# XuyangBai/D3Feat

Measured on NVIDIA H100. Metric: points/sec through KPFCNN encoder, higher is better.
Workload: dtype f32

## Files before the change

d3feat_b200/csrc/kpconv.cu:

```cuda
#include <stdlib.h>

#include "ops.cuh"

namespace d3f {


constexpr int kS1Warps = 4;
constexpr int kWStride = 20;
constexpr int kKMax = 16;

struct Stage1Params {
  const float* q;
  const float4* s4;
  const int* idx;
  const float* feat;
  int count_nn;
  const float* Kp;
  const float* offsets;
  const float* modulations;
  int Nq, Ns, H, Cin;
  int n0, n1;
  const int* order;
  float extent;
  float inv_scale;
// ... 200 lines not shown
__device__ __forceinline__ float sqrt_approx(float x) {
  float r;
  asm("sqrt.approx.ftz.f32 %0, %1;" : "=f"(r) : "f"(x));
  return r;
}

template <int CPL, int QPW, bool DEFORM>
__global__ void __launch_bounds__(kS1Warps * 32, CPL == 4 ? 4 : 6) kpconv_stage1_v2_kernel(Stage1Params p) {
  const int Ns_ = dyn_rows(p.Ns, p.ns_dev), n1_ = min(p.n1, dyn_rows(p.Nq, p.nq_dev));
  constexpr int K = 15, KP = 16;
  constexpr int LPQ = 32 / QPW;
  static_assert(CPL == 2 || CPL == 4, "channels per lane");
  __shared__ __align__(16) float wts[kS1Warps][32 * kWStride];
  __shared__ float kp_s[kS1Warps][QPW][KP * 3];
  const int lane = threadIdx.x & 31, warp = threadIdx.x >> 5;
  const int sub = lane / LPQ, sl = lane % LPQ;
  const int nfirst = p.n0 + (blockIdx.x * kS1Warps + warp) * QPW;
  if (nfirst >= n1_) return;
  const int n = nfirst + sub;
  const bool qvalid = n < n1_;
  const int nslot = qvalid ? n : nfirst;
  const int nq = p.order ? p.order[nslot] : nslot;

  for (int t = sl; t < KP * 3; t += LPQ) {
    float v = t < K * 3 ? p.Kp[t] : 0.f;
    if (DEFORM && t < K * 3) v += p.offsets[(size_t)nq * K * 3 + t];
    kp_s[warp][sub][t] = v;
  }
  const float qx = p.q[3 * (size_t)nq], qy = p.q[3 * (size_t)nq + 1], qz = p.q[3 * (size_t)nq + 2];
  const int* row = p.idx + (size_t)nq * p.H;
  const float ext2 = p.extent * p.extent;
  const unsigned gshift = (unsigned)(sub * LPQ);
  const unsigned gmask = LPQ == 32 ? 0xffffffffu : ((1u << LPQ) - 1u);
  float* wq = &wts[warp][sub * LPQ * kWStride];
  __syncwarp();

  int nn_count = 0;
  constexpr int c_step = LPQ * CPL;
  for (int c0 = 0; c0 < p.Cin; c0 += c_step) {
    float2 acc[KP / 2][CPL];
#pragma unroll
    for (int j = 0; j < KP / 2; ++j)
#pragma unroll
      for (int v = 0; v < CPL; ++v) acc[j][v] = make_float2(0.f, 0.f);
    const int c = c0 + sl * CPL;

    for (int h0 = 0; h0 < p.H; h0 += LPQ) {
      const int h = h0 + sl;
      int id = (h < p.H) ? row[h] : Ns_;
      if (id < 0 || id > Ns_) id = Ns_;
      const bool real = id < Ns_;
      const float4 sp = __ldg(&p.s4[id]);
      const float rx = sp.x - qx, ry = sp.y - qy, rz = sp.z - qz;
      float w[KP];
      float dmin = 3.0e38f;
      int kmin = 0;
      bool in_range = false;
#pragma unroll
      for (int k = 0; k < K; ++k) {
        float dx = rx - kp_s[warp][sub][3 * k], dy = ry - kp_s[warp][sub][3 * k + 1], dz = rz - kp_s[warp][sub][3 * k + 2];
        float d2 = dx * dx + dy * dy + dz * dz;
        if (d2 < dmin) { dmin = d2; kmin = k; }
        in_range = in_range || (d2 < ext2);
        float wk;
        if (p.influence == D3F_INFLUENCE_LINEAR) wk = fmaxf(1.f - sqrt_approx(d2 + 1e-10f) * p.inv_scale, 0.f);
        else if (p.influence == D3F_INFLUENCE_GAUSSIAN) wk = __expf(-d2 * p.gauss_inv);
        else wk = DEFORM ? (d2 < ext2 ? 1.f : 0.f) : 1.f;
        w[k] = wk;
      }
      w[K] = 0.f;
      if (p.closest) {
#pragma unroll
        for (int k = 0; k < K; ++k) w[k] = (k == kmin) ? w[k] : 0.f;
      }
      const bool keep = real && qvalid && (!DEFORM || in_range);
#pragma unroll
      for (int kq = 0; kq < KP / 4; ++kq)
        *reinterpret_cast<float4*>(&wq[sl * kWStride + 4 * kq]) =
            keep ? make_float4(w[4 * kq], w[4 * kq + 1], w[4 * kq + 2], w[4 * kq + 3]) : make_float4(0.f, 0.f, 0.f, 0.f);
      if (c0 == 0 && p.count_nn) nn_count += __popc((__ballot_sync(0xffffffffu, sp.w > 0.f) >> gshift) & gmask);
      unsigned m = (__ballot_sync(0xffffffffu, keep) >> gshift) & gmask;
      int cnt = __popc(m);
      if (QPW >= 2) cnt = max(cnt, __shfl_xor_sync(0xffffffffu, cnt, 16));
      if (QPW >= 4) cnt = max(cnt, __shfl_xor_sync(0xffffffffu, cnt, 8));
      __syncwarp();

      constexpr int kUnroll = CPL == 4 ? 2 : 4;
      for (int it = 0; it < cnt; it += kUnroll) {
        int hh[kUnroll];
        float f[kUnroll][CPL];
#pragma unroll
        for (int u = 0; u < kUnroll; ++u) {
          const bool act = m != 0;
          hh[u] = act ? __ffs(m) - 1 : 0;
          m &= m - 1;
          const int idh = __shfl_sync(0xffffffffu, id, (int)gshift + hh[u]);
          const float* fp = p.feat + (size_t)idh * p.Cin + c;
          if (CPL == 4) {
            float4 t = act ? __ldg(reinterpret_cast<const float4*>(fp)) : make_float4(0.f, 0.f, 0.f, 0.f);
            f[u][0] = t.x; f[u][1] = t.y; f[u][2 % CPL] = t.z; f[u][3 % CPL] = t.w;
          } else {
            float2 t = act ? __ldg(reinterpret_cast<const float2*>(fp)) : make_float2(0.f, 0.f);
            f[u][0] = t.x; f[u][1] = t.y;
          }
        }
#pragma unroll
        for (int u = 0; u < kUnroll; ++u) {
          const float4* wp = reinterpret_cast<const float4*>(&wq[hh[u] * kWStride]);
          float2 wpair[KP / 2];
#pragma unroll
          for (int kq = 0; kq < KP / 4; ++kq) {
            float4 t = wp[kq];
            wpair[2 * kq] = make_float2(t.x, t.y);
            wpair[2 * kq + 1] = make_float2(t.z, t.w);
          }
#pragma unroll
          for (int v = 0; v < CPL; ++v) {
            const float2 fd = make_float2(f[u][v], f[u][v]);
#pragma unroll
            for (int j = 0; j < KP / 2; ++j) acc[j][v] = ffma2(wpair[j], fd, acc[j][v]);
          }
        }
      }
      __syncwarp();
    }

    if (qvalid) {
      float* dst = p.wf + (size_t)(n - p.n0) * K * p.Cin + c;
#pragma unroll
      for (int k = 0; k < K; ++k) {
        const float mod = (DEFORM && p.modulations) ? p.modulations[(size_t)nq * K + k] : 1.f;
        float o[CPL];
#pragma unroll
        for (int v = 0; v < CPL; ++v) o[v] = ((k & 1) ? acc[k / 2][v].y : acc[k / 2][v].x) * mod;
        if (CPL == 4) *reinterpret_cast<float4*>(dst + (size_t)k * p.Cin) = make_float4(o[0], o[1], o[2 % CPL], o[3 % CPL]);
        else *reinterpret_cast<float2*>(dst + (size_t)k * p.Cin) = make_float2(o[0], o[1]);
      }
    }
  }
  if (p.inv_nn != nullptr && qvalid && sl == 0) p.inv_nn[n - p.n0] = 1.f / (float)max(nn_count, 1);
}

__device__ __forceinline__ void mma_tf32(float (&c)[4], const unsigned (&a)[4], unsigned b0, unsigned b1) {
  asm volatile("mma.sync.aligned.m16n8k8.row.col.f32.tf32.tf32.f32 {%0,%1,%2,%3}, {%4,%5,%6,%7}, {%8,%9}, {%0,%1,%2,%3};"
               : "+f"(c[0]), "+f"(c[1]), "+f"(c[2]), "+f"(c[3])
               : "r"(a[0]), "r"(a[1]), "r"(a[2]), "r"(a[3]), "r"(b0), "r"(b1));
}
__device__ __forceinline__ void split3(float x, unsigned& hi, unsigned& lo) {
  hi = (__float_as_uint(x) + 0x1000u) & 0xFFFFE000u;
  lo = __float_as_uint(x - __uint_as_float(hi));
}


template <int NT>
__global__ void __launch_bounds__(kS1Warps * 32, NT == 4 ? 8 : (NT == 8 ? 5 : 3))
kpconv_stage1_fast_kernel(Stage1Params p) {
  const int Ns_ = dyn_rows(p.Ns, p.ns_dev), n1_ = min(p.n1, dyn_rows(p.Nq, p.nq_dev));
  constexpr int K = 15;
  static_assert(NT % 4 == 0, "one float4 per four n-tiles");
  const int lane = threadIdx.x & 31, warp = threadIdx.x >> 5;
  const int g = lane >> 2, t = lane & 3;
  const int n = p.n0 + blockIdx.x * kS1Warps + warp;
  if (n >= n1_) return;
  const int kA = g, kB = g + 8;
  const bool validB = kB < K;
  const float kax = p.Kp[3 * kA], kay = p.Kp[3 * kA + 1], kaz = p.Kp[3 * kA + 2];
  const float kbx = validB ? p.Kp[3 * kB] : 1e6f, kby = validB ? p.Kp[3 * kB + 1] : 1e6f,
              kbz = validB ? p.Kp[3 * kB + 2] : 1e6f;
  const int qid = p.order ? p.order[n] : n;
  const float qx = p.q[3 * (size_t)qid], qy = p.q[3 * (size_t)qid + 1], qz = p.q[3 * (size_t)qid + 2];
  const int* row = p.idx + (size_t)qid * p.H + t;
  const float inv_scale = p.inv_scale;
  const unsigned Ns = (unsigned)Ns_;
  const unsigned Cin = (unsigned)p.Cin;
  int cnt = 0;

  constexpr int CCH = NT * 8;
  for (int c0 = blockIdx.y * CCH; c0 < p.Cin; c0 += gridDim.y * CCH) {
    float acc[NT][4];
#pragma unroll
    for (int i = 0; i < NT; ++i) acc[i][0] = acc[i][1] = acc[i][2] = acc[i][3] = 0.f;
    const float* fcol = p.feat + c0 + NT * g;
    asm volatile("" : "+l"(fcol));

    unsigned ida_n = Ns, idb_n = Ns;
    if (t < p.H) ida_n = (unsigned)__ldg(row);
    if (t + 4 < p.H) idb_n = (unsigned)__ldg(row + 4);
    for (int h0 = 0; h0 < p.H; h0 += 8) {
      const unsigned ida = min(ida_n, Ns);
      const unsigned idb = min(idb_n, Ns);
      ida_n = Ns;
      idb_n = Ns;
      if (h0 + 8 + t < p.H) ida_n = (unsigned)__ldg(row + h0 + 8);
      if (h0 + 12 + t < p.H) idb_n = (unsigned)__ldg(row + h0 + 12);
      const float4 spa = __ldg(&p.s4[ida]), spb = __ldg(&p.s4[idb]);
      float fa[NT], fb[NT];
#pragma unroll
      for (int v = 0; v < NT; v += 4) {
        float4 x = make_float4(0.f, 0.f, 0.f, 0.f), y = make_float4(0.f, 0.f, 0.f, 0.f);
        if (ida < Ns) x = __ldg(reinterpret_cast<const float4*>(fcol + (size_t)(ida * Cin) + v));
        if (idb < Ns) y = __ldg(reinterpret_cast<const float4*>(fcol + (size_t)(idb * Cin) + v));
        fa[v] = x.x; fa[v + 1] = x.y; fa[v + 2] = x.z; fa[v + 3] = x.w;
        fb[v] = y.x; fb[v + 1] = y.y; fb[v + 2] = y.z; fb[v + 3] = y.w;
      }
      if (c0 == 0) cnt += (spa.w > 0.f ? 1 : 0) + (spb.w > 0.f ? 1 : 0);
      const float rax = spa.x - qx, ray = spa.y - qy, raz = spa.z - qz;
      const float rbx = spb.x - qx, rby = spb.y - qy, rbz = spb.z - qz;
      auto weight = [&](float rx, float ry, float rz, float kx, float ky, float kz) {
        const float dx = rx - kx, dy = ry - ky, dz = rz - kz;
        const float d2 = fmaf(dz, dz, fmaf(dy, dy, fmaf(dx, dx, 1e-10f)));
        return fmaxf(fmaf(-sqrt_approx(d2), inv_scale, 1.f), 0.f);
      };
      unsigned ah[4], al[4];
      split3(weight(rax, ray, raz, kax, kay, kaz), ah[0], al[0]);
      split3(weight(rax, ray, raz, kbx, kby, kbz), ah[1], al[1]);
      split3(weight(rbx, rby, rbz, kax, kay, kaz), ah[2], al[2]);
      split3(weight(rbx, rby, rbz, kbx, kby, kbz), ah[3], al[3]);
#pragma unroll
      for (int i = 0; i < NT; ++i) {
        unsigned bh0, bl0, bh1, bl1;
        split3(fa[i], bh0, bl0);
        split3(fb[i], bh1, bl1);
        mma_tf32(acc[i], ah, bh0, bh1);
        mma_tf32(acc[i], al, bh0, bh1);
        mma_tf32(acc[i], ah, bl0, bl1);
      }
    }

    float* dst = p.wf + (size_t)(n - p.n0) * K * p.Cin + c0 + 2 * NT * t;
#pragma unroll
    for (int v = 0; v < NT; v += 4) {
      *reinterpret_cast<float4*>(dst + (size_t)kA * p.Cin + v) = make_float4(acc[v][0], acc[v + 1][0], acc[v + 2][0], acc[v + 3][0]);
      *reinterpret_cast<float4*>(dst + (size_t)kA * p.Cin + NT + v) = make_float4(acc[v][1], acc[v + 1][1], acc[v + 2][1], acc[v + 3][1]);
      if (validB) {
        *reinterpret_cast<float4*>(dst + (size_t)kB * p.Cin + v) = make_float4(acc[v][2], acc[v + 1][2], acc[v + 2][2], acc[v + 3][2]);
        *reinterpret_cast<float4*>(dst + (size_t)kB * p.Cin + NT + v) = make_float4(acc[v][3], acc[v + 1][3], acc[v + 2][3], acc[v + 3][3]);
      }
    }
  }
  if (p.inv_nn != nullptr && blockIdx.y == 0) {
    cnt += __shfl_xor_sync(0xffffffffu, cnt, 1);
    cnt += __shfl_xor_sync(0xffffffffu, cnt, 2);
    if (lane == 0) p.inv_nn[n - p.n0] = 1.f / (float)max(cnt, 1);
  }
}

__device__ __forceinline__ uint32_t s1_smem_u32(const void* p) { return (uint32_t)__cvta_generic_to_shared(p); }
__device__ __forceinline__ void s1_cp_async16(uint32_t dst, const void* src, bool valid) {
  const int sz = valid ? 16 : 0;
  asm volatile("cp.async.cg.shared.global [%0], [%1], 16, %2;" ::"r"(dst), "l"(src), "r"(sz) : "memory");
}
__device__ __forceinline__ float4 s1_lds128(uint32_t addr) {
  float4 v;
  asm volatile("ld.shared.v4.f32 {%0, %1, %2, %3}, [%4];" : "=f"(v.x), "=f"(v.y), "=f"(v.z), "=f"(v.w) : "r"(addr));
  return v;
}
template <int NT>
__device__ __forceinline__ int s1_swz(int r3) {
  return NT == 4 ? 2 * r3 : (NT == 8 ? ((r3 & 1) | ((r3 & 2) << 1)) : r3);
}

template <int NT>
__global__ void __launch_bounds__(kS1Warps * 32, NT == 4 ? 8 : (NT == 8 ? 5 : 3))
kpconv_stage1_staged_kernel(Stage1Params p) {
  constexpr int K = 15;
  constexpr int ROWB = NT * 32;
  constexpr int BUFB = 8 * ROWB + 128;
  __shared__ __align__(128) unsigned char stage_sm[kS1Warps][2][BUFB];
  const int Ns_ = dyn_rows(p.Ns, p.ns_dev), n1_ = min(p.n1, dyn_rows(p.Nq, p.nq_dev));
  const int lane = threadIdx.x & 31, warp = threadIdx.x >> 5;
  const int g = lane >> 2, t = lane & 3;
  const int n = p.n0 + blockIdx.x * kS1Warps + warp;
  if (n >= n1_) return;
  const int kA = g, kB = g + 8;
  const bool validB = kB < K;
  const float kax = p.Kp[3 * kA], kay = p.Kp[3 * kA + 1], kaz = p.Kp[3 * kA + 2];
  const float kbx = validB ? p.Kp[3 * kB] : 1e6f, kby = validB ? p.Kp[3 * kB + 1] : 1e6f,
              kbz = validB ? p.Kp[3 * kB + 2] : 1e6f;
  const int qid = p.order ? p.order[n] : n;
  const float qx = p.q[3 * (size_t)qid], qy = p.q[3 * (size_t)qid + 1], qz = p.q[3 * (size_t)qid + 2];
  const int* rowq = p.idx + (size_t)qid * p.H;
  const float inv_scale = p.inv_scale;
  const unsigned Ns = (unsigned)Ns_;
  const unsigned Cin = (unsigned)p.Cin;
  const uint32_t base = s1_smem_u32(&stage_sm[warp][0][0]);
  const int cr = lane >> 3, cc = lane & 7;
  uint32_t wr_row = (uint32_t)(cr * ROWB + (cc ^ s1_swz<NT>(cr & 3)) * 16);
  uint32_t wr_s4 = (uint32_t)(8 * ROWB + lane * 16);
  uint32_t rd_s4 = (uint32_t)(8 * ROWB + t * 16);
  uint32_t rd_row[NT / 4];
#pragma unroll
  for (int v = 0; v < NT; v += 4) {
    const int chunk = g * (NT / 4) + v / 4;
    rd_row[v / 4] = (uint32_t)(t * ROWB + (chunk & ~7) * 16 + (((chunk & 7) ^ s1_swz<NT>(t)) * 16));
    asm volatile("" : "+r"(rd_row[v / 4]));
  }
  asm volatile("" : "+r"(wr_row), "+r"(wr_s4), "+r"(rd_s4));
  int cnt = 0;

  constexpr int CCH = NT * 8;
  for (int c0 = blockIdx.y * CCH; c0 < p.Cin; c0 += gridDim.y * CCH) {
    float acc[NT][4];
#pragma unroll
    for (int i = 0; i < NT; ++i) acc[i][0] = acc[i][1] = acc[i][2] = acc[i][3] = 0.f;
    const float* fsrc = p.feat + c0 + 4 * cc;
    asm volatile("" : "+l"(fsrc));
    auto load_ids = [&](int h0) -> unsigned {
      unsigned v = Ns;
      if (lane < 8 && h0 + lane < p.H) v = (unsigned)__ldg(rowq + h0 + lane);
      return min(v, Ns);
    };
    auto issue = [&](unsigned idv, uint32_t buf) {
      if (lane < 8) s1_cp_async16(buf + wr_s4, p.s4 + idv, true);
      const unsigned i0 = __shfl_sync(0xffffffffu, idv, cr), i1 = __shfl_sync(0xffffffffu, idv, cr + 4);
      const bool ok0 = i0 < Ns, ok1 = i1 < Ns;
      const float* s0 = fsrc + (size_t)((ok0 ? i0 : 0u) * Cin);
      const float* s1 = fsrc + (size_t)((ok1 ? i1 : 0u) * Cin);
#pragma unroll
      for (int seg = 0; seg < ROWB / 128; ++seg) {
        s1_cp_async16(buf + wr_row + seg * 128, s0 + seg * 32, ok0);
        s1_cp_async16(buf + wr_row + 4 * ROWB + seg * 128, s1 + seg * 32, ok1);
      }
    };
    uint32_t cur = base, nxt = base + BUFB;
    unsigned idv_n = load_ids(0);
    issue(idv_n, cur);
    asm volatile("cp.async.commit_group;" ::: "memory");
    idv_n = load_ids(8);
    for (int h0 = 0; h0 < p.H; h0 += 8) {
      if (h0 + 8 < p.H) issue(idv_n, nxt);
      asm volatile("cp.async.commit_group;" ::: "memory");
      idv_n = load_ids(h0 + 16);
      asm volatile("cp.async.wait_group 1;" ::: "memory");
      __syncwarp();
      const float4 spa = s1_lds128(cur + rd_s4), spb = s1_lds128(cur + rd_s4 + 64);
      float fa[NT], fb[NT];
#pragma unroll
      for (int v = 0; v < NT; v += 4) {
        const float4 x = s1_lds128(cur + rd_row[v / 4]), y = s1_lds128(cur + rd_row[v / 4] + 4 * ROWB);
        fa[v] = x.x; fa[v + 1] = x.y; fa[v + 2] = x.z; fa[v + 3] = x.w;
        fb[v] = y.x; fb[v + 1] = y.y; fb[v + 2] = y.z; fb[v + 3] = y.w;
      }
      if (c0 == 0) cnt += (spa.w > 0.f ? 1 : 0) + (spb.w > 0.f ? 1 : 0);
      const float rax = spa.x - qx, ray = spa.y - qy, raz = spa.z - qz;
      const float rbx = spb.x - qx, rby = spb.y - qy, rbz = spb.z - qz;
      auto weight = [&](float rx, float ry, float rz, float kx, float ky, float kz) {
        const float dx = rx - kx, dy = ry - ky, dz = rz - kz;
        const float d2 = fmaf(dz, dz, fmaf(dy, dy, fmaf(dx, dx, 1e-10f)));
        return fmaxf(fmaf(-sqrt_approx(d2), inv_scale, 1.f), 0.f);
      };
      unsigned ah[4], al[4];
      split3(weight(rax, ray, raz, kax, kay, kaz), ah[0], al[0]);
      split3(weight(rax, ray, raz, kbx, kby, kbz), ah[1], al[1]);
      split3(weight(rbx, rby, rbz, kax, kay, kaz), ah[2], al[2]);
      split3(weight(rbx, rby, rbz, kbx, kby, kbz), ah[3], al[3]);
#pragma unroll
      for (int i = 0; i < NT; ++i) {
        unsigned bh0, bl0, bh1, bl1;
        split3(fa[i], bh0, bl0);
        split3(fb[i], bh1, bl1);
        mma_tf32(acc[i], ah, bh0, bh1);
        mma_tf32(acc[i], al, bh0, bh1);
        mma_tf32(acc[i], ah, bl0, bl1);
      }
      __syncwarp();
      const uint32_t tmp = cur;
      cur = nxt;
      nxt = tmp;
    }
    asm volatile("cp.async.wait_group 0;" ::: "memory");

    float* dst = p.wf + (size_t)(n - p.n0) * K * p.Cin + c0 + 2 * NT * t;
#pragma unroll
    for (int v = 0; v < NT; v += 4) {
      *reinterpret_cast<float4*>(dst + (size_t)kA * p.Cin + v) = make_float4(acc[v][0], acc[v + 1][0], acc[v + 2][0], acc[v + 3][0]);
      *reinterpret_cast<float4*>(dst + (size_t)kA * p.Cin + NT + v) = make_float4(acc[v][1], acc[v + 1][1], acc[v + 2][1], acc[v + 3][1]);
      if (validB) {
        *reinterpret_cast<float4*>(dst + (size_t)kB * p.Cin + v) = make_float4(acc[v][2], acc[v + 1][2], acc[v + 2][2], acc[v + 3][2]);
        *reinterpret_cast<float4*>(dst + (size_t)kB * p.Cin + NT + v) = make_float4(acc[v][3], acc[v + 1][3], acc[v + 2][3], acc[v + 3][3]);
      }
// ... 209 lines not shown

template <bool DEFORM>
static int launch_stage1(int K, const Stage1Params& p, cudaStream_t stream) {
  int nq = p.n1 - p.n0;
  bool al16 = (reinterpret_cast<uintptr_t>(p.feat) & 15) == 0 && (reinterpret_cast<uintptr_t>(p.wf) & 15) == 0;
  if (K == 15 && al16 && (p.Cin == 32 || p.Cin == 64 || p.Cin % 128 == 0)) {
    const int blocks = ceil_div(nq, kS1Warps);
    const bool fast = p.influence == D3F_INFLUENCE_LINEAR && !p.closest;
    static const bool no_pared = [] { const char* v = getenv("D3F_S1_PARED"); return v != nullptr && v[0] == '0'; }();
    if (fast && !DEFORM && !no_pared && (long long)(p.Ns + 1) * p.Cin < (1ll << 31)) {
      const char* sv = getenv("D3F_S1_STAGED");
      const int staged = sv ? atoi(sv) : 0;
      const dim3 grid_wide(blocks, p.Cin >= 128 ? p.Cin / 64 : 1);
      if (staged) {
        if (p.Cin == 32) kpconv_stage1_staged_kernel<4><<<blocks, kS1Warps * 32, 0, stream>>>(p);
        else kpconv_stage1_staged_kernel<8><<<grid_wide, kS1Warps * 32, 0, stream>>>(p);
        D3F_LAUNCH_CHECK("kpconv_stage1_staged_kernel");
        return D3F_OK;
      }
      if (p.Cin == 32) kpconv_stage1_fast_kernel<4><<<blocks, kS1Warps * 32, 0, stream>>>(p);
      else kpconv_stage1_fast_kernel<8><<<grid_wide, kS1Warps * 32, 0, stream>>>(p);
      D3F_LAUNCH_CHECK("kpconv_stage1_fast_kernel");
      return D3F_OK;
    }
    if (fast) {
      if (p.Cin == 32) kpconv_stage1_mma_kernel<4, DEFORM, true><<<blocks, kS1Warps * 32, 0, stream>>>(p);
      else if (p.Cin == 64) kpconv_stage1_mma_kernel<8, DEFORM, true><<<blocks, kS1Warps * 32, 0, stream>>>(p);
      else kpconv_stage1_mma_kernel<16, DEFORM, true><<<blocks, kS1Warps * 32, 0, stream>>>(p);
    } else {
      if (p.Cin == 32) kpconv_stage1_mma_kernel<4, DEFORM, false><<<blocks, kS1Warps * 32, 0, stream>>>(p);
      else if (p.Cin == 64) kpconv_stage1_mma_kernel<8, DEFORM, false><<<blocks, kS1Warps * 32, 0, stream>>>(p);
      else kpconv_stage1_mma_kernel<16, DEFORM, false><<<blocks, kS1Warps * 32, 0, stream>>>(p);
    }
    D3F_LAUNCH_CHECK("kpconv_stage1_mma_kernel");
    return D3F_OK;
  }
  if (K == 15 && al16 && p.Cin % 64 == 0) {
    kpconv_stage1_v2_kernel<2, 1, DEFORM><<<ceil_div(nq, kS1Warps), kS1Warps * 32, 0, stream>>>(p);
  } else if (K == 15 && al16 && p.Cin % 32 == 0) {
    kpconv_stage1_v2_kernel<2, 2, DEFORM><<<ceil_div(nq, kS1Warps * 2), kS1Warps * 32, 0, stream>>>(p);
  } else if (K == 15) {
    kpconv_stage1_kernel<15, 1, DEFORM><<<ceil_div(nq, kS1Warps), kS1Warps * 32, 0, stream>>>(p);
  } else {
    const size_t smem = (size_t)kS1Warps * (K * 32 + K * 3) * sizeof(float);
    kpconv_stage1_anyk_kernel<DEFORM><<<ceil_div(nq, kS1Warps), kS1Warps * 32, smem, stream>>>(p, K);
  }
  D3F_LAUNCH_CHECK("kpconv_stage1_kernel");
  return D3F_OK;
}

struct Cin1Params {
  const float* q; const float4* s4; const int* idx; const float* Kp; const float* W;
  int Nq, Ns, H, Cout;
  float inv_scale, gauss_inv;
  int influence, closest, normalize;
  float shadow;
  const float* bn_scale; const float* bn_shift; const float* bias;
  float leaky_alpha;
  const int* order;
  float* out;
  const int* nq_dev; const int* ns_dev;
};

template <bool FAST>
__global__ void __launch_bounds__(256, 3) kpconv_cin1_kernel(Cin1Params p) {
  const int Ns_ = dyn_rows(p.Ns, p.ns_dev), Nq_ = dyn_rows(p.Nq, p.nq_dev);
  constexpr int K = 15;
  extern __shared__ float c1_smem[];
  float* Ws = c1_smem;
  float* kp_s = c1_smem + K * p.Cout;
  for (int t = threadIdx.x; t < K * p.Cout; t += blockDim.x) Ws[t] = p.W[t];
  for (int t = threadIdx.x; t < K * 3; t += blockDim.x) kp_s[t] = p.Kp[t];
  __syncthreads();
  const int lane = threadIdx.x & 31;
  const int sub = lane >> 3, sl = lane & 7;
  const int slot0 = ((blockIdx.x * blockDim.x + threadIdx.x) >> 5) * 4;
  if (slot0 >= Nq_) return;
  const int slot = slot0 + sub;
  const bool qvalid = slot < Nq_;
  const int n = p.order ? p.order[qvalid ? slot : slot0] : (qvalid ? slot : slot0);
  const float qx = p.q[3 * (size_t)n], qy = p.q[3 * (size_t)n + 1], qz = p.q[3 * (size_t)n + 2];
  const int* row = p.idx + (size_t)n * p.H;
  float wf[K];
#pragma unroll
  for (int k = 0; k < K; ++k) wf[k] = 0.f;
  int nn = 0;
  if (FAST) {
    float kp[K * 3];
#pragma unroll
    for (int i = 0; i < K * 3; ++i) kp[i] = kp_s[i];
    const float inv_scale = p.inv_scale;
    const unsigned Nsu = (unsigned)Ns_;
    unsigned id1 = Nsu, id2 = Nsu;
    if (sl < p.H) id1 = min((unsigned)__ldg(row + sl), Nsu);
    if (sl + 8 < p.H) id2 = min((unsigned)__ldg(row + sl + 8), Nsu);
    float4 sp_n = __ldg(&p.s4[id1]);
    for (int h = sl; h < p.H; h += 8) {
      const float4 sp = sp_n;
      sp_n = __ldg(&p.s4[id2]);
      id2 = Nsu;
      if (h + 16 < p.H) id2 = min((unsigned)__ldg(row + h + 16), Nsu);
      const float f = sp.w, rx = sp.x - qx, ry = sp.y - qy, rz = sp.z - qz;
      nn += f > 0.f ? 1 : 0;
#pragma unroll
      for (int k = 0; k < K; ++k) {
        const float dx = rx - kp[3 * k], dy = ry - kp[3 * k + 1], dz = rz - kp[3 * k + 2];
        const float d2 = fmaf(dz, dz, fmaf(dy, dy, fmaf(dx, dx, 1e-10f)));
        const float wk = fmaxf(fmaf(-sqrt_approx(d2), inv_scale, 1.f), 0.f);
        wf[k] = fmaf(wk, f, wf[k]);
      }
    }
  } else
  for (int h = sl; h < p.H; h += 8) {
    int id = row[h];
    if (id < 0 || id > Ns_) id = Ns_;
    const float4 sp = __ldg(&p.s4[id]);
    const float f = sp.w, rx = sp.x - qx, ry = sp.y - qy, rz = sp.z - qz;
    nn += f > 0.f ? 1 : 0;
    float w[K];
    float dmin = 3.0e38f;
    int kmin = 0;
#pragma unroll
    for (int k = 0; k < K; ++k) {
      float dx = rx - kp_s[3 * k], dy = ry - kp_s[3 * k + 1], dz = rz - kp_s[3 * k + 2];
      float d2 = dx * dx + dy * dy + dz * dz;
      if (d2 < dmin) { dmin = d2; kmin = k; }
      float wk;
      if (p.influence == D3F_INFLUENCE_LINEAR) wk = fmaxf(1.f - sqrt_approx(d2 + 1e-10f) * p.inv_scale, 0.f);
      else if (p.influence == D3F_INFLUENCE_GAUSSIAN) wk = __expf(-d2 * p.gauss_inv);
      else wk = 1.f;
      w[k] = wk;
    }
#pragma unroll
    for (int k = 0; k < K; ++k) wf[k] += (p.closest && k != kmin) ? 0.f : w[k] * f;
  }
#pragma unroll
  for (int o = 1; o < 8; o <<= 1) {
#pragma unroll
    for (int k = 0; k < K; ++k) wf[k] += __shfl_xor_sync(0xffffffffu, wf[k], o);
    nn += __shfl_xor_sync(0xffffffffu, nn, o);
  }
  if (!qvalid) return;
  const float inv_nn = p.normalize ? 1.f / (float)max(nn, 1) : 1.f;
  for (int c = sl; c < p.Cout; c += 8) {
    float y = 0.f;
#pragma unroll
    for (int k = 0; k < K; ++k) y = fmaf(wf[k], Ws[k * p.Cout + c], y);
    y *= inv_nn;
    if (p.bn_scale) y = fmaf(y, p.bn_scale[c], p.bn_shift[c]);
    if (p.bias) y += p.bias[c];
    if (p.leaky_alpha >= 0.f) y = y > 0.f ? y : y * p.leaky_alpha;
    p.out[(size_t)n * p.Cout + c] = y;
  }
}

struct AuxStream {
  cudaStream_t stream = nullptr;
  cudaEvent_t s1_done[2] = {nullptr, nullptr};
  cudaEvent_t gemm_done[2] = {nullptr, nullptr};
};
constexpr int kMaxDevices = 32;
struct AuxStreams {
  AuxStream dev[kMaxDevices];
  ~AuxStreams() {
    for (int d = 0; d < kMaxDevices; ++d) {
      if (dev[d].stream == nullptr) continue;
      int cur = 0;
      if (cudaGetDevice(&cur) != cudaSuccess || cudaSetDevice(d) != cudaSuccess) continue;
      for (int i = 0; i < 2; ++i) {
        cudaEventDestroy(dev[d].s1_done[i]);
        cudaEventDestroy(dev[d].gemm_done[i]);
      }
      cudaStreamDestroy(dev[d].stream);
      cudaSetDevice(cur);
    }
  }
};
static AuxStream* aux_stream() {
  static thread_local AuxStreams all;
  int dev = 0;
  if (cudaGetDevice(&dev) != cudaSuccess || dev < 0 || dev >= kMaxDevices) return nullptr;
  AuxStream& a = all.dev[dev];
  if (a.stream != nullptr) return &a;
  if (cudaStreamCreateWithFlags(&a.stream, cudaStreamNonBlocking) != cudaSuccess) { a.stream = nullptr; return nullptr; }
  for (int i = 0; i < 2; ++i) {
    cudaEventCreateWithFlags(&a.s1_done[i], cudaEventDisableTiming);
    cudaEventCreateWithFlags(&a.gemm_done[i], cudaEventDisableTiming);
  }
  return &a;
}

static int chunk_queries(int K, int Cin) {
  static const int forced = [] { const char* v = getenv("D3F_KPCONV_CHUNK"); return v ? atoi(v) : 0; }();
  if (forced >= 128) return forced / 128 * 128;
  const long long per = (long long)K * Cin * 4;
  long long n = (512ll << 20) / per;
  if (n < 1024) n = 1024;
  return (int)(n / 128 * 128);
}

size_t kpconv_workspace_bytes(int Nq, int Ns, int H, int K, int Cin, int Cout) {
  (void)H; (void)Cout;
  int chunk = chunk_queries(K, Cin);
  if (chunk > Nq) chunk = Nq > 0 ? Nq : 1;
  size_t b = 0;
  b += 2 * align_up((size_t)chunk * K * Cin * sizeof(float), 256);
  b += 2 * align_up((size_t)chunk * sizeof(float), 256);
  b += align_up((size_t)(Ns + 1) * sizeof(float4), 256);
  b += align_up(tc_gemm_split_ws_floats(chunk, Cout, K * Cin) * sizeof(float), 256);
  b += align_up(kpconv_fused_workspace_bytes(), 256);
  return b + 1024;
}

int kpconv_forward_impl(bool deform, const float* q, const float* s, const int* idx, const float* feat,
                        const float* Kp, const float* offsets, const float* modulations, const float* W,
                        const float* W_packed, const int* query_order, int Nq, int Ns, int H, int K, int Cin, int Cout,
                        float extent,
                        int influence, int mode, int normalize,
                        const float* bn_scale, const float* bn_shift, const float* bias, float leaky_alpha,
                        float* out, void* workspace, size_t workspace_bytes, cudaStream_t stream,
                        const int* nq_dev, const int* ns_dev) {
  D3F_REQUIRE(Nq >= 0 && Ns >= 0 && H >= 0 && Cin >= 1 && Cout >= 1, D3F_ERR_INVALID,
              "kpconv: bad shape Nq=%d Ns=%d H=%d Cin=%d Cout=%d", Nq, Ns, H, Cin, Cout);
  D3F_REQUIRE(K >= 1 && K <= kAnyKMax, D3F_ERR_INVALID, "kpconv: num_kernel_points=%d outside [1, %d]", K, kAnyKMax);
  D3F_REQUIRE(influence >= 0 && influence <= 2, D3F_ERR_INVALID,
              "Unknown influence function type (config.KP_influence)");
  D3F_REQUIRE(mode == D3F_MODE_SUM || mode == D3F_MODE_CLOSEST, D3F_ERR_INVALID,
              "Unknown convolution mode. Should be 'closest' or 'sum'");
  D3F_REQUIRE(extent > 0.f, D3F_ERR_INVALID, "kpconv: KP_extent=%g", (double)extent);
  D3F_REQUIRE((bn_scale == nullptr) == (bn_shift == nullptr), D3F_ERR_INVALID, "kpconv: bn_scale/bn_shift mismatch");
  D3F_REQUIRE(!deform || offsets != nullptr || Nq == 0, D3F_ERR_INVALID, "kpconv_deform: offsets missing");
  D3F_REQUIRE(workspace_bytes >= kpconv_workspace_bytes(Nq, Ns, H, K, Cin, Cout), D3F_ERR_WORKSPACE,
              "kpconv: workspace too small");
  if (Nq == 0) return D3F_OK;
  int chunk = chunk_queries(K, Cin);
  if (chunk > Nq) chunk = Nq;
  Carver cv(workspace, workspace_bytes);
  float* wf_buf[2] = {cv.take<float>((size_t)chunk * K * Cin), cv.take<float>((size_t)chunk * K * Cin)};
  float* nn_buf[2] = {cv.take<float>(chunk), cv.take<float>(chunk)};
  float4* s4 = cv.take<float4>((size_t)Ns + 1);
  size_t split_floats = tc_gemm_split_ws_floats(chunk, Cout, K * Cin);
  float* split_ws = split_floats ? cv.take<float>(split_floats) : nullptr;
  const bool norm = normalize != 0 && !deform;
  {
    const bool first_layer = Cin == 1 && !deform && K == 15;
    int pmode = first_layer ? 2 : (norm ? 1 : 0);
    const float shadow = deform ? 1000.f : 1e6f;
    const bool vec = pmode == 1 && Cin % 4 == 0 && Cin >= 32 && (reinterpret_cast<uintptr_t>(feat) & 15) == 0;
    if (vec && Cin < 64)
      prep_supports_vec_kernel<8><<<ceil_div((Ns + 1) * 8, 256), 256, 0, stream>>>(s, feat, Ns, ns_dev, Cin, shadow, s4);
    else if (vec && Cin < 128)
      prep_supports_vec_kernel<16><<<ceil_div((Ns + 1) * 16, 256), 256, 0, stream>>>(s, feat, Ns, ns_dev, Cin, shadow, s4);
    else if (vec)
      prep_supports_vec_kernel<32><<<ceil_div((Ns + 1) * 32, 256), 256, 0, stream>>>(s, feat, Ns, ns_dev, Cin, shadow, s4);
    else
      prep_supports_kernel<<<ceil_div((Ns + 1) * 32, 256), 256, 0, stream>>>(s, feat, Ns, ns_dev, Cin, pmode, shadow, s4);
    D3F_LAUNCH_CHECK("prep_supports_kernel");
  }
  if (Cin == 1 && !deform && K == 15) {
    Cin1Params c1;
    c1.q = q; c1.s4 = s4; c1.idx = idx; c1.Kp = Kp; c1.W = W;
    c1.Nq = Nq; c1.Ns = Ns; c1.H = H; c1.Cout = Cout;
    c1.inv_scale = 1.f / (2.f * extent);
    float sg = extent * 0.3f;
    c1.gauss_inv = 1.f / (2.f * sg * sg + 1e-9f);
    c1.influence = influence; c1.closest = mode == D3F_MODE_CLOSEST; c1.normalize = normalize != 0;
    c1.shadow = 1e6f;
    c1.bn_scale = bn_scale; c1.bn_shift = bn_shift; c1.bias = bias; c1.leaky_alpha = leaky_alpha;
    c1.order = query_order;
    c1.out = out;
    c1.nq_dev = nq_dev; c1.ns_dev = ns_dev;
    const size_t c1_smem = (size_t)(K * Cout + K * 3) * sizeof(float);
    D3F_REQUIRE(c1_smem <= 48 * 1024, D3F_ERR_CAPACITY, "kpconv (Cin = 1): Cout=%d too wide for the first-layer kernel", Cout);
    if (influence == D3F_INFLUENCE_LINEAR && mode == D3F_MODE_SUM)
      kpconv_cin1_kernel<true><<<ceil_div(ceil_div(Nq, 4) * 32, 256), 256, c1_smem, stream>>>(c1);
    else
      kpconv_cin1_kernel<false><<<ceil_div(ceil_div(Nq, 4) * 32, 256), 256, c1_smem, stream>>>(c1);
    D3F_LAUNCH_CHECK("kpconv_cin1_kernel");
    return D3F_OK;
  }
  if (!deform && W_packed != nullptr &&
      kpconv_fused_supported(Nq, H, K, Cin, Cout, influence, mode, feat, W, out, query_order)) {
    float* w_img = cv.take<float>(kpconv_fused_workspace_bytes() / sizeof(float));
    return kpconv_fused_forward(q, s4, idx, feat, Kp, W, w_img, Nq, Ns, H, Cout, extent, norm ? 1 : 0, bn_scale, bn_shift,
                                bias, leaky_alpha, out, stream, nq_dev, ns_dev);
  }
  Stage1Params p;
  p.q = q; p.s4 = s4; p.idx = idx; p.feat = feat; p.count_nn = norm ? 1 : 0;
  p.Kp = Kp; p.offsets = offsets; p.modulations = modulations;
  p.Nq = Nq; p.Ns = Ns; p.H = H; p.Cin = Cin;
  p.extent = extent;
  p.inv_scale = deform ? 1.f / extent : 1.f / (2.f * extent);
  float sigma = extent * 0.3f;
  p.gauss_inv = 1.f / (2.f * sigma * sigma + 1e-9f);
  p.influence = influence;
  p.closest = mode == D3F_MODE_CLOSEST;
  p.shadow = deform ? 1000.f : 1e6f;
  p.order = query_order;
  p.nq_dev = nq_dev; p.ns_dev = ns_dev;
  const int n_chunks = ceil_div(Nq, chunk);
  AuxStream* aux = n_chunks > 1 ? aux_stream() : nullptr;
  for (int ci = 0, n0 = 0; n0 < Nq; n0 += chunk, ++ci) {
    const int b = ci & 1;
    float* wf = wf_buf[b];
    float* inv_nn = nn_buf[b];
    p.wf = wf;
    p.inv_nn = norm ? inv_nn : nullptr;
    p.n0 = n0;
    p.n1 = min(Nq, n0 + chunk);
    if (aux && ci >= 2) D3F_CUDA(cudaStreamWaitEvent(stream, aux->gemm_done[b], 0));
    int rc = deform ? launch_stage1<true>(K, p, stream) : launch_stage1<false>(K, p, stream);
    if (rc) return rc;
    cudaStream_t gs = stream;
    if (aux) {
      D3F_CUDA(cudaEventRecord(aux->s1_done[b], stream));
      D3F_CUDA(cudaStreamWaitEvent(aux->stream, aux->s1_done[b], 0));
      gs = aux->stream;
    }
    Epilogue ep;
    ep.rowscale = norm ? inv_nn : nullptr;
    ep.bn_scale = bn_scale; ep.bn_shift = bn_shift; ep.bias = bias; ep.residual = nullptr;
    ep.leaky_alpha = leaky_alpha;
    ep.row_map = query_order ? query_order + n0 : nullptr;
    ep.m_dev = nq_dev; ep.m_off = n0;
    float* cbase = query_order ? out : out + (size_t)n0 * Cout;
    if (W_packed != nullptr && tc_gemm_supported(wf, K * Cin))
      rc = tc_gemm(wf, W_packed, cbase, p.n1 - n0, Cout, K * Cin, ep, gs, split_ws);
    else
      rc = gemm_f32(wf, W, cbase, p.n1 - n0, Cout, K * Cin, ep, gs);
    if (rc) return rc;
    if (aux) D3F_CUDA(cudaEventRecord(aux->gemm_done[b], aux->stream));
  }
  if (aux) {
    D3F_CUDA(cudaStreamWaitEvent(stream, aux->gemm_done[0], 0));
    if (n_chunks > 1) D3F_CUDA(cudaStreamWaitEvent(stream, aux->gemm_done[1], 0));
  }
  return D3F_OK;
}

}
```

Baseline: 52.66 million.

## Fuse KPConv stage1 weighting and weight GEMM into one shared-memory tile kernel

Adds a fused kernel for rigid linear-sum KPConv with Cin==Cout in {32,64}. Each block computes the weighted neighbor features for a tile of queries into shared memory using the existing stage1 MMA pass. It then multiplies that tile by W with 3xTF32 MMAs, reduces the partial sums across warps and applies normalization, BN, bias and leaky ReLU in the epilogue. This removes the global wf buffer round trip, the chunked two-stream pipeline and the separate GEMM launch, at the cost of heavy shared memory per block and reading W from global memory in every block.

```diff
diff --git a/d3feat_b200/csrc/kpconv.cu b/d3feat_b200/csrc/kpconv.cu
--- a/d3feat_b200/csrc/kpconv.cu
+++ b/d3feat_b200/csrc/kpconv.cu
@@ -376,80 +376,96 @@
 }
 
 
+struct FastKp {
+  float ax, ay, az, bx, by, bz;
+};
+__device__ __forceinline__ FastKp fast_kernel_points(const float* Kp, int g) {
+  const int kA = g, kB = g + 8;
+  const bool validB = kB < 15;
+  return FastKp{Kp[3 * kA], Kp[3 * kA + 1], Kp[3 * kA + 2], validB ? Kp[3 * kB] : 1e6f,
+                validB ? Kp[3 * kB + 1] : 1e6f, validB ? Kp[3 * kB + 2] : 1e6f};
+}
+
+template <int NT>
+__device__ __forceinline__ void stage1_fast_pass(const Stage1Params& p, const int* row, unsigned Ns, int c0, int g,
+                                                 float qx, float qy, float qz, const FastKp& kp, float (&acc)[NT][4],
+                                                 int& cnt) {
+  static_assert(NT % 4 == 0, "one float4 per four n-tiles");
+  const float kax = kp.ax, kay = kp.ay, kaz = kp.az, kbx = kp.bx, kby = kp.by, kbz = kp.bz;
+  const float inv_scale = p.inv_scale;
+  const unsigned Cin = (unsigned)p.Cin;
+  const int t = threadIdx.x & 3;
+#pragma unroll
+  for (int i = 0; i < NT; ++i) acc[i][0] = acc[i][1] = acc[i][2] = acc[i][3] = 0.f;
+  const float* fcol = p.feat + c0 + NT * g;
+  asm volatile("" : "+l"(fcol));
+
+  unsigned ida_n = Ns, idb_n = Ns;
+  if (t < p.H) ida_n = (unsigned)__ldg(row);
+  if (t + 4 < p.H) idb_n = (unsigned)__ldg(row + 4);
+  for (int h0 = 0; h0 < p.H; h0 += 8) {
+    const unsigned ida = min(ida_n, Ns);
+    const unsigned idb = min(idb_n, Ns);
+    ida_n = Ns;
+    idb_n = Ns;
+    if (h0 + 8 + t < p.H) ida_n = (unsigned)__ldg(row + h0 + 8);
+    if (h0 + 12 + t < p.H) idb_n = (unsigned)__ldg(row + h0 + 12);
+    const float4 spa = __ldg(&p.s4[ida]), spb = __ldg(&p.s4[idb]);
+    float fa[NT], fb[NT];
+#pragma unroll
+    for (int v = 0; v < NT; v += 4) {
+      float4 x = make_float4(0.f, 0.f, 0.f, 0.f), y = make_float4(0.f, 0.f, 0.f, 0.f);
+      if (ida < Ns) x = __ldg(reinterpret_cast<const float4*>(fcol + (size_t)(ida * Cin) + v));
+      if (idb < Ns) y = __ldg(reinterpret_cast<const float4*>(fcol + (size_t)(idb * Cin) + v));
+      fa[v] = x.x; fa[v + 1] = x.y; fa[v + 2] = x.z; fa[v + 3] = x.w;
+      fb[v] = y.x; fb[v + 1] = y.y; fb[v + 2] = y.z; fb[v + 3] = y.w;
+    }
+    if (c0 == 0) cnt += (spa.w > 0.f ? 1 : 0) + (spb.w > 0.f ? 1 : 0);
+    const float rax = spa.x - qx, ray = spa.y - qy, raz = spa.z - qz;
+    const float rbx = spb.x - qx, rby = spb.y - qy, rbz = spb.z - qz;
+    auto weight = [&](float rx, float ry, float rz, float kx, float ky, float kz) {
+      const float dx = rx - kx, dy = ry - ky, dz = rz - kz;
+      const float d2 = fmaf(dz, dz, fmaf(dy, dy, fmaf(dx, dx, 1e-10f)));
+      return fmaxf(fmaf(-sqrt_approx(d2), inv_scale, 1.f), 0.f);
+    };
+    unsigned ah[4], al[4];
+    split3(weight(rax, ray, raz, kax, kay, kaz), ah[0], al[0]);
+    split3(weight(rax, ray, raz, kbx, kby, kbz), ah[1], al[1]);
+    split3(weight(rbx, rby, rbz, kax, kay, kaz), ah[2], al[2]);
+    split3(weight(rbx, rby, rbz, kbx, kby, kbz), ah[3], al[3]);
+#pragma unroll
+    for (int i = 0; i < NT; ++i) {
+      unsigned bh0, bl0, bh1, bl1;
+      split3(fa[i], bh0, bl0);
+      split3(fb[i], bh1, bl1);
+      mma_tf32(acc[i], ah, bh0, bh1);
+      mma_tf32(acc[i], al, bh0, bh1);
+      mma_tf32(acc[i], ah, bl0, bl1);
+    }
+  }
+}
+
 template <int NT>
 __global__ void __launch_bounds__(kS1Warps * 32, NT == 4 ? 8 : (NT == 8 ? 5 : 3))
 kpconv_stage1_fast_kernel(Stage1Params p) {
   const int Ns_ = dyn_rows(p.Ns, p.ns_dev), n1_ = min(p.n1, dyn_rows(p.Nq, p.nq_dev));
   constexpr int K = 15;
-  static_assert(NT % 4 == 0, "one float4 per four n-tiles");
   const int lane = threadIdx.x & 31, warp = threadIdx.x >> 5;
   const int g = lane >> 2, t = lane & 3;
   const int n = p.n0 + blockIdx.x * kS1Warps + warp;
   if (n >= n1_) return;
   const int kA = g, kB = g + 8;
   const bool validB = kB < K;
-  const float kax = p.Kp[3 * kA], kay = p.Kp[3 * kA + 1], kaz = p.Kp[3 * kA + 2];
-  const float kbx = validB ? p.Kp[3 * kB] : 1e6f, kby = validB ? p.Kp[3 * kB + 1] : 1e6f,
-              kbz = validB ? p.Kp[3 * kB + 2] : 1e6f;
+  const FastKp kp = fast_kernel_points(p.Kp, g);
   const int qid = p.order ? p.order[n] : n;
   const float qx = p.q[3 * (size_t)qid], qy = p.q[3 * (size_t)qid + 1], qz = p.q[3 * (size_t)qid + 2];
   const int* row = p.idx + (size_t)qid * p.H + t;
-  const float inv_scale = p.inv_scale;
-  const unsigned Ns = (unsigned)Ns_;
-  const unsigned Cin = (unsigned)p.Cin;
   int cnt = 0;
 
   constexpr int CCH = NT * 8;
   for (int c0 = blockIdx.y * CCH; c0 < p.Cin; c0 += gridDim.y * CCH) {
     float acc[NT][4];
-#pragma unroll
-    for (int i = 0; i < NT; ++i) acc[i][0] = acc[i][1] = acc[i][2] = acc[i][3] = 0.f;
-    const float* fcol = p.feat + c0 + NT * g;
-    asm volatile("" : "+l"(fcol));
-
-    unsigned ida_n = Ns, idb_n = Ns;
-    if (t < p.H) ida_n = (unsigned)__ldg(row);
-    if (t + 4 < p.H) idb_n = (unsigned)__ldg(row + 4);
-    for (int h0 = 0; h0 < p.H; h0 += 8) {
-      const unsigned ida = min(ida_n, Ns);
-      const unsigned idb = min(idb_n, Ns);
-      ida_n = Ns;
-      idb_n = Ns;
-      if (h0 + 8 + t < p.H) ida_n = (unsigned)__ldg(row + h0 + 8);
-      if (h0 + 12 + t < p.H) idb_n = (unsigned)__ldg(row + h0 + 12);
-      const float4 spa = __ldg(&p.s4[ida]), spb = __ldg(&p.s4[idb]);
-      float fa[NT], fb[NT];
-#pragma unroll
-      for (int v = 0; v < NT; v += 4) {
-        float4 x = make_float4(0.f, 0.f, 0.f, 0.f), y = make_float4(0.f, 0.f, 0.f, 0.f);
-        if (ida < Ns) x = __ldg(reinterpret_cast<const float4*>(fcol + (size_t)(ida * Cin) + v));
-        if (idb < Ns) y = __ldg(reinterpret_cast<const float4*>(fcol + (size_t)(idb * Cin) + v));
-        fa[v] = x.x; fa[v + 1] = x.y; fa[v + 2] = x.z; fa[v + 3] = x.w;
-        fb[v] = y.x; fb[v + 1] = y.y; fb[v + 2] = y.z; fb[v + 3] = y.w;
-      }
-      if (c0 == 0) cnt += (spa.w > 0.f ? 1 : 0) + (spb.w > 0.f ? 1 : 0);
-      const float rax = spa.x - qx, ray = spa.y - qy, raz = spa.z - qz;
-      const float rbx = spb.x - qx, rby = spb.y - qy, rbz = spb.z - qz;
-      auto weight = [&](float rx, float ry, float rz, float kx, float ky, float kz) {
-        const float dx = rx - kx, dy = ry - ky, dz = rz - kz;
-        const float d2 = fmaf(dz, dz, fmaf(dy, dy, fmaf(dx, dx, 1e-10f)));
-        return fmaxf(fmaf(-sqrt_approx(d2), inv_scale, 1.f), 0.f);
-      };
-      unsigned ah[4], al[4];
-      split3(weight(rax, ray, raz, kax, kay, kaz), ah[0], al[0]);
-      split3(weight(rax, ray, raz, kbx, kby, kbz), ah[1], al[1]);
-      split3(weight(rbx, rby, rbz, kax, kay, kaz), ah[2], al[2]);
-      split3(weight(rbx, rby, rbz, kbx, kby, kbz), ah[3], al[3]);
-#pragma unroll
-      for (int i = 0; i < NT; ++i) {
-        unsigned bh0, bl0, bh1, bl1;
-        split3(fa[i], bh0, bl0);
-        split3(fb[i], bh1, bl1);
-        mma_tf32(acc[i], ah, bh0, bh1);
-        mma_tf32(acc[i], al, bh0, bh1);
-        mma_tf32(acc[i], ah, bl0, bl1);
-      }
-    }
+    stage1_fast_pass<NT>(p, row, (unsigned)Ns_, c0, g, qx, qy, qz, kp, acc, cnt);
 
     float* dst = p.wf + (size_t)(n - p.n0) * K * p.Cin + c0 + 2 * NT * t;
 #pragma unroll
@@ -965,6 +981,189 @@
     if (p.leaky_alpha >= 0.f) y = y > 0.f ? y : y * p.leaky_alpha;
     p.out[(size_t)n * p.Cout + c] = y;
   }
+}
+
+struct FusedTileParams {
+  Stage1Params s1;
+  const float* W;
+  const float* bn_scale; const float* bn_shift; const float* bias;
+  float leaky_alpha;
+  float* out;
+};
+
+constexpr int kFtWarps = 8;
+template <int NT> struct FusedTile {
+  static constexpr int kCin = 8 * NT;
+  static constexpr int kTQ = NT == 4 ? 32 : 16;
+  static constexpr int kKc = 15 * kCin;
+  static constexpr int kLd = kKc + 4;
+  static constexpr int kMinCtas = NT == 4 ? 3 : 2;
+  static constexpr size_t kSmem = (size_t)kTQ * kLd * sizeof(float) + kTQ * sizeof(float);
+  static_assert((kTQ / 16) * (kCin / 8) == kFtWarps, "one 16 x 8 output block per warp");
+  static_assert(kMinCtas * (kSmem + 1024) <= 233472, "shared memory of an H100 SM");
+};
+
+template <int NT>
+__global__ void __launch_bounds__(kFtWarps * 32, FusedTile<NT>::kMinCtas) kpconv_fused_tile_kernel(FusedTileParams fp) {
+  using T = FusedTile<NT>;
+  constexpr int CIN = T::kCin, TQ = T::kTQ, LD = T::kLd;
+  const Stage1Params& p = fp.s1;
+  const int Nq_ = dyn_rows(p.Nq, p.nq_dev);
+  const int slot0 = blockIdx.x * TQ;
+  if (slot0 >= Nq_) return;
+  extern __shared__ __align__(16) float ft_smem[];
+  float* wf_s = ft_smem;
+  float* inv_nn_s = ft_smem + TQ * LD;
+  const int lane = threadIdx.x & 31, warp = threadIdx.x >> 5;
+  const int g = lane >> 2, t = lane & 3;
+
+  {
+    const unsigned Ns = (unsigned)dyn_rows(p.Ns, p.ns_dev);
+    const FastKp kp = fast_kernel_points(p.Kp, g);
+    const int kA = g, kB = g + 8;
+    for (int r = warp; r < TQ; r += kFtWarps) {
+      const int n = slot0 + r;
+      float* dst = wf_s + r * LD + 2 * NT * t;
+      if (n >= Nq_) {
+#pragma unroll
+        for (int v = 0; v < 2 * NT; v += 4) {
+          *reinterpret_cast<float4*>(dst + kA * CIN + v) = make_float4(0.f, 0.f, 0.f, 0.f);
+          if (kB < 15) *reinterpret_cast<float4*>(dst + kB * CIN + v) = make_float4(0.f, 0.f, 0.f, 0.f);
+        }
+        continue;
+      }
+      const int qid = p.order ? p.order[n] : n;
+      const float qx = p.q[3 * (size_t)qid], qy = p.q[3 * (size_t)qid + 1], qz = p.q[3 * (size_t)qid + 2];
+      float acc[NT][4];
+      int cnt = 0;
+      stage1_fast_pass<NT>(p, p.idx + (size_t)qid * p.H + t, Ns, 0, g, qx, qy, qz, kp, acc, cnt);
+#pragma unroll
+      for (int v = 0; v < NT; v += 4) {
+        *reinterpret_cast<float4*>(dst + kA * CIN + v) = make_float4(acc[v][0], acc[v + 1][0], acc[v + 2][0], acc[v + 3][0]);
+        *reinterpret_cast<float4*>(dst + kA * CIN + NT + v) = make_float4(acc[v][1], acc[v + 1][1], acc[v + 2][1], acc[v + 3][1]);
+        if (kB < 15) {
+          *reinterpret_cast<float4*>(dst + kB * CIN + v) = make_float4(acc[v][2], acc[v + 1][2], acc[v + 2][2], acc[v + 3][2]);
+          *reinterpret_cast<float4*>(dst + kB * CIN + NT + v) = make_float4(acc[v][3], acc[v + 1][3], acc[v + 2][3], acc[v + 3][3]);
+        }
+      }
+      cnt += __shfl_xor_sync(0xffffffffu, cnt, 1);
+      cnt += __shfl_xor_sync(0xffffffffu, cnt, 2);
+      if (lane == 0) inv_nn_s[r] = p.count_nn ? 1.f / (float)max(cnt, 1) : 1.f;
+    }
+  }
+  __syncthreads();
+
+  constexpr int MT = TQ / 16, NO = CIN / 8, NCH = T::kKc / 32;
+  constexpr int NH = 2, KG = kFtWarps / NH, NW = NO / NH;
+  const int kg = warp % KG, j0 = (warp / KG) * NW;
+  float part[MT][NW][4];
+#pragma unroll
+  for (int m = 0; m < MT; ++m)
+#pragma unroll
+    for (int j = 0; j < NW; ++j) part[m][j][0] = part[m][j][1] = part[m][j][2] = part[m][j][3] = 0.f;
+  const float* a_base = wf_s + g * LD + t;
+  const float* b_base = fp.W + 8 * j0 + g + (size_t)t * CIN;
+  for (int ch = kg; ch < NCH; ch += KG) {
+    float acc[MT][NW][4];
+#pragma unroll
+    for (int m = 0; m < MT; ++m)
+#pragma unroll
+      for (int j = 0; j < NW; ++j) acc[m][j][0] = acc[m][j][1] = acc[m][j][2] = acc[m][j][3] = 0.f;
+#pragma unroll
+    for (int s = 0; s < 4; ++s) {
+      const int k = 32 * ch + 8 * s;
+      unsigned ah[MT][4], al[MT][4];
+#pragma unroll
+      for (int m = 0; m < MT; ++m) {
+        const float* a = a_base + 16 * m * LD + k;
+        split3(a[0], ah[m][0], al[m][0]);
+        split3(a[8 * LD], ah[m][1], al[m][1]);
+        split3(a[4], ah[m][2], al[m][2]);
+        split3(a[8 * LD + 4], ah[m][3], al[m][3]);
+      }
+#pragma unroll
+      for (int j = 0; j < NW; ++j) {
+        unsigned bh0, bl0, bh1, bl1;
+        split3(__ldg(b_base + (size_t)k * CIN + 8 * j), bh0, bl0);
+        split3(__ldg(b_base + (size_t)(k + 4) * CIN + 8 * j), bh1, bl1);
+#pragma unroll
+        for (int m = 0; m < MT; ++m) {
+          mma_tf32(acc[m][j], ah[m], bh0, bh1);
+          mma_tf32(acc[m][j], al[m], bh0, bh1);
+          mma_tf32(acc[m][j], ah[m], bl0, bl1);
+        }
+      }
+    }
+#pragma unroll
+    for (int m = 0; m < MT; ++m)
+#pragma unroll
+      for (int j = 0; j < NW; ++j)
+#pragma unroll
+        for (int i = 0; i < 4; ++i) part[m][j][i] += acc[m][j][i];
+  }
+
+  static_assert(KG * MT * NO * 4 * 32 <= TQ * LD, "partials fit in the wf tile");
+  static_assert(MT * NO * 2 * 32 == 2 * kFtWarps * 32, "two fragment pairs per thread");
+  float2* red_s = reinterpret_cast<float2*>(wf_s);
+  __syncthreads();
+#pragma unroll
+  for (int m = 0; m < MT; ++m)
+#pragma unroll
+    for (int j = 0; j < NW; ++j)
+#pragma unroll
+      for (int h = 0; h < 2; ++h)
+        red_s[((kg * MT + m) * NO + j0 + j) * 64 + h * 32 + lane] = make_float2(part[m][j][2 * h], part[m][j][2 * h + 1]);
+  __syncthreads();
+#pragma unroll
+  for (int u = 0; u < 2; ++u) {
+    const int e = threadIdx.x + u * kFtWarps * 32;
+    const int el = e & 31, h = (e >> 5) & 1, mj = e >> 6;
+    const int r = 16 * (mj / NO) + (el >> 2) + 8 * h, col = 8 * (mj % NO) + 2 * (el & 3);
+    float2 y = red_s[e];
+#pragma unroll
+    for (int w = 1; w < KG; ++w) {
+      const float2 v = red_s[w * MT * NO * 64 + e];
+      y.x += v.x;
+      y.y += v.y;
+    }
+    const int n = slot0 + r;
+    if (n >= Nq_) continue;
+    const float rs = inv_nn_s[r];
+    float o[2] = {y.x * rs, y.y * rs};
+#pragma unroll
+    for (int c = 0; c < 2; ++c) {
+      if (fp.bn_scale) o[c] = fmaf(o[c], fp.bn_scale[col + c], fp.bn_shift[col + c]);
+      if (fp.bias) o[c] += fp.bias[col + c];
+      if (fp.leaky_alpha >= 0.f) o[c] = o[c] > 0.f ? o[c] : o[c] * fp.leaky_alpha;
+    }
+    const size_t orow = p.order ? (size_t)p.order[n] : (size_t)n;
+    *reinterpret_cast<float2*>(fp.out + orow * CIN + col) = make_float2(o[0], o[1]);
+  }
+}
+
+static bool fused_tile_eligible(int Nq, int Ns, int K, int Cin, int Cout, int influence, int mode, const float* feat,
+                                const float* out) {
+  constexpr int kMinQueries = 8192;
+  if (!(K == 15 && influence == D3F_INFLUENCE_LINEAR && mode == D3F_MODE_SUM && (Cin == 32 || Cin == 64) &&
+        Cout == Cin && Nq >= kMinQueries && (long long)(Ns + 1) * Cin < (1ll << 31) &&
+        (reinterpret_cast<uintptr_t>(feat) & 15) == 0 && (reinterpret_cast<uintptr_t>(out) & 7) == 0))
+    return false;
+  for (const char* v : {"D3F_FUSED_KPCONV", "D3F_S1_STAGED", "D3F_KPCONV_CHUNK", "D3F_S1_PARED"})
+    if (getenv(v) != nullptr) return false;
+  return true;
+}
+
+template <int NT>
+static int launch_fused_tile(const FusedTileParams& fp, cudaStream_t stream) {
+  using T = FusedTile<NT>;
+  static bool configured = false;
+  if (!configured) {
+    D3F_CUDA(cudaFuncSetAttribute(kpconv_fused_tile_kernel<NT>, cudaFuncAttributeMaxDynamicSharedMemorySize, (int)T::kSmem));
+    configured = true;
+  }
+  kpconv_fused_tile_kernel<NT><<<ceil_div(fp.s1.Nq, T::kTQ), kFtWarps * 32, T::kSmem, stream>>>(fp);
+  D3F_LAUNCH_CHECK("kpconv_fused_tile_kernel");
+  return D3F_OK;
 }
 
 struct AuxStream {
@@ -1111,6 +1310,15 @@
   p.shadow = deform ? 1000.f : 1e6f;
   p.order = query_order;
   p.nq_dev = nq_dev; p.ns_dev = ns_dev;
+  if (!deform && fused_tile_eligible(Nq, Ns, K, Cin, Cout, influence, mode, feat, out)) {
+    p.count_nn = norm ? 1 : 0;
+    p.wf = nullptr; p.inv_nn = nullptr; p.n0 = 0; p.n1 = Nq;
+    FusedTileParams fp;
+    fp.s1 = p; fp.W = W;
+    fp.bn_scale = bn_scale; fp.bn_shift = bn_shift; fp.bias = bias; fp.leaky_alpha = leaky_alpha;
+    fp.out = out;
+    return Cin == 32 ? launch_fused_tile<4>(fp, stream) : launch_fused_tile<8>(fp, stream);
+  }
   const int n_chunks = ceil_div(Nq, chunk);
   AuxStream* aux = n_chunks > 1 ? aux_stream() : nullptr;
   for (int ci = 0, n0 = 0; n0 < Nq; n0 += chunk, ++ci) {
```

Measured after the change: 54.81 million, median of 6. 4.1% higher.
